# MJavaadAkhtar/GCN-max-cut

Measured on AMD Instinct MI355X. Metric: training epochs/sec (n=1000 d=7 graphs), higher is better.
Workload: dtype f32; 1 GPU; 160 x n=1000 d=7 regular graphs per GPU (BASELINE configs[3] on one GPU; 160 graphs per step), GCN 1000->500->3, batched steps, Adam lr 1e-3; graphs_per_gpu=160, rows_per_gpu=160000, nnz_per_gpu=1120000, hidden_dim=500, mode=batched, epoch_graphs=160, parallelism=single

## Files before the change

gcn-max-cut_amd/csrc/bwd1_lds.hip:

```cpp
#include "lds_tile.h"
#include "head_body.h"

#ifdef GMC_STAMP
extern "C" int gmc_debug_read_stamps_bwd(unsigned long long *out, int n) {
    return (int)hipMemcpyFromSymbol(out, HIP_SYMBOL(g_stamps), sizeof(unsigned long long) * n);
}
extern "C" int gmc_debug_read_stamps_bwdhead(unsigned long long *out, int n) {
    return (int)hipMemcpyFromSymbol(out, HIP_SYMBOL(g_hstamps), sizeof(unsigned long long) * n);
}
#endif

namespace {

struct Bwd1Args {
    gmc_batch b;
    const float *H;
    const float *GY2;
    const float *W2;
    float *dw1part;
    float *colpart;
    int F;
    int slices;
    int chunks;
    int graphs_per_chunk;
    int ovf_cap;
    int own_lds;
    const float *hZ0;
    int hzparts;
    float hC;
    const float *hb2;
    float *hP;
    int *hS;
    float *hloss;
    float *hdb2part;
    int *htick;
};

struct ColState {
    gmc::v2f w2p[2][3];
    gmc::v2f cdw2[3][2], cdb1[2];
};

__device__ __forceinline__ void col_state_init(ColState &c, const float *W2, int f0, bool col_on) {
#pragma unroll
    for (int p = 0; p < 2; ++p) {
#pragma unroll
        for (int k = 0; k < 3; ++k) {
            c.w2p[p][k] = col_on ? (gmc::v2f){W2[(long)(f0 + 2 * p) * 3 + k], W2[(long)(f0 + 2 * p + 1) * 3 + k]}
                                 : gmc::splat2(0.f);
            c.cdw2[k][p] = gmc::splat2(0.f);
        }
        c.cdb1[p] = gmc::splat2(0.f);
    }
}

__device__ __forceinline__ void transform_row(ColState &c, float4 *cell, const float4 rck, const float4 *hreg = nullptr) {
    const float d = rck.w;
    const float4 h = hreg ? *hreg : *cell;
    const gmc::v2f g0 = gmc::splat2(rck.x * d), g1 = gmc::splat2(rck.y * d), g2 = gmc::splat2(rck.z * d);
    const gmc::v2f hp[2] = {{h.x, h.y}, {h.z, h.w}};
    gmc::v2f gs[2];
#pragma unroll
    for (int p = 0; p < 2; ++p) {
        gmc::v2f ghd = g0 * c.w2p[p][0];
        ghd = gmc::pk_fma(g1, c.w2p[p][1], ghd);
        ghd = gmc::pk_fma(g2, c.w2p[p][2], ghd);
        const gmc::v2f gpre = {hp[p].x > 0.f ? ghd.x : 0.f, hp[p].y > 0.f ? ghd.y : 0.f};
        gs[p] = gpre * gmc::splat2(d);
        if (ABL(3)) continue;
        c.cdw2[0][p] = gmc::pk_fma(hp[p], g0, c.cdw2[0][p]);
        c.cdw2[1][p] = gmc::pk_fma(hp[p], g1, c.cdw2[1][p]);
        c.cdw2[2][p] = gmc::pk_fma(hp[p], g2, c.cdw2[2][p]);
        c.cdb1[p] += gpre;
    }
    *cell = make_float4(gs[0].x, gs[0].y, gs[1].x, gs[1].y);
#pragma unroll
    for (int p = 0; p < 2; ++p)
        asm volatile("" : "+v"(c.cdw2[0][p]), "+v"(c.cdw2[1][p]), "+v"(c.cdw2[2][p]), "+v"(c.cdb1[p]));
}

template <int Q>
__device__ __forceinline__ void col_epilogue(const ColState &c, float *red, float *colpart, int chunk, int s, int FS, int F) {
    float colp[16];
#pragma unroll
    for (int p = 0; p < 2; ++p) {
#pragma unroll
        for (int k = 0; k < 3; ++k) { colp[4 * (2 * p) + k] = c.cdw2[k][p].x; colp[4 * (2 * p + 1) + k] = c.cdw2[k][p].y; }
        colp[4 * (2 * p) + 3] = c.cdb1[p].x; colp[4 * (2 * p + 1) + 3] = c.cdb1[p].y;
    }
#pragma unroll
    for (int i = 0; i < 16; ++i) colp[i] = gmc::xor_tree<32, Q>(colp[i]);
    const int wave = threadIdx.x >> 6, lane = threadIdx.x & 63;
    if (lane < Q) {
#pragma unroll
        for (int i = 0; i < 16; ++i) red[(wave * Q + lane) * 16 + i] = colp[i];
    }
    lds_barrier();
    if (threadIdx.x < Q * 4) {
        const int qq = threadIdx.x / 4, j = threadIdx.x % 4;
        if (s * FS + 4 * qq < F) {
            float o[4] = {0.f, 0.f, 0.f, 0.f};
            for (int wv = 0; wv < kThreads / 64; ++wv)
#pragma unroll
                for (int cc = 0; cc < 4; ++cc) o[cc] += red[(wv * Q + qq) * 16 + 4 * j + cc];
            reinterpret_cast<float4 *>(colpart)[(long)chunk * F + s * FS + 4 * qq + j] = make_float4(o[0], o[1], o[2], o[3]);
        }
    }
}

__device__ __forceinline__ void dma_row_consts(const float *GY2, int r0, int n, float *gyl) {
    const unsigned base = (unsigned)(size_t)(__attribute__((address_space(3))) float *)gyl;
    int tid = threadIdx.x;
    asm volatile("" : "+v"(tid));
    for (int i0 = 0; i0 < n; i0 += kThreads) {
        const unsigned dst = (unsigned)__builtin_amdgcn_readfirstlane((int)(base + 16u * (unsigned)(i0 + (tid & ~63))));
        if (i0 + tid < n) glds16(GY2 + (long)(r0 + i0 + tid) * 4, dst);
    }
}

template <int FS, int ACC, bool HAS_VAL, int NS, bool OVF, bool HEAD = false>
__global__ GMC_LDS_BOUNDS void bwd1_reg_kernel(Bwd1Args a) {
    extern __shared__ __attribute__((aligned(16))) float lds[];
    constexpr int W = 8;
    constexpr int Q = FS / 4;
    constexpr int kRowsPerPass = kThreads / Q;
    int chunk, s;
    MARK(0);
    tile_of((int)blockIdx.x, a.chunks, a.slices, chunk, s);
    const int TF = (int)tile_floats(a.b.n_max, FS);
    float *bufA = lds, *bufB = lds + TF;
    float *gy0 = lds + 2 * TF + (size_t)a.b.n_max * W / 2;
    float *gy1 = lds + 2 * TF;
    float *red = bufB;
    const int q = threadIdx.x % Q, lrow = threadIdx.x / Q;
    const int f0 = s * FS + 4 * q;
    const bool col_on = f0 < a.F;
    const float *Hs = a.H + (long)s * a.b.R * FS;
    ColState cs;
    col_state_init(cs, a.W2, f0, col_on);
    gmc::v4f acc[ACC];
#pragma unroll
    for (int k = 0; k < ACC; ++k) acc[k] = (gmc::v4f)(0.f);

    const int g0 = chunk * a.graphs_per_chunk, g1 = min(a.b.B, g0 + a.graphs_per_chunk);
    if (g0 >= g1) return;
    constexpr bool ovf = OVF;

    constexpr bool kRecycle = !HAS_VAL && !OVF;
    constexpr int KREG = kRecycle ? 3 : 0;
    float4 hreg[kRecycle ? KREG : 1];
    auto load_cell = [&](int slot, int k, int r0n, int nn) {
        const int l = min(lrow + k * kRowsPerPass, nn - 1);
        const gmc::v4f v = __builtin_nontemporal_load(reinterpret_cast<const gmc::v4f *>(Hs + (long)(r0n + l) * FS + 4 * q));
        hreg[slot] = make_float4(v.x, v.y, v.z, v.w);
    };
    auto load_hreg = [&](int r0n, int nn) {
#pragma unroll
        for (int k = 0; k < KREG; ++k) {
            const int l = min(lrow + k * kRowsPerPass, nn - 1);
            const gmc::v4f v = __builtin_nontemporal_load(reinterpret_cast<const gmc::v4f *>(Hs + (long)(r0n + l) * FS + 4 * q));
            hreg[k] = make_float4(v.x, v.y, v.z, v.w);
        }
    };
    uint4 idr[ACC];
    OvfLds ol{};
    constexpr int kOvfRows = (ACC * kRowsPerPass + kThreads - 1) / kThreads;
    OvfReq<kOvfRows> orq;
    if constexpr (ovf) ol = ovf_lds(lds, a.own_lds, a.b.n_max, a.ovf_cap);
    auto load_ids = [&](int r0, int n) {
#pragma unroll
        for (int k = 0; k < ACC; ++k)
            idr[k] = *reinterpret_cast<const uint4 *>(a.b.ell + (long)(r0 + min(lrow + k * kRowsPerPass, n - 1)) * W);
    };
    auto pad_ids = [&](int n) {
        const unsigned pad = (unsigned)n * 0x10001u;
#pragma unroll
        for (int k = 0; k < ACC; ++k)
            if (lrow + k * kRowsPerPass >= n) idr[k] = make_uint4(pad, pad, pad, pad);
    };
    auto zero_pads = [&](float *buf, int n) {
        if (threadIdx.x < kPadRows * FS) buf[n * FS + threadIdx.x] = 0.f;
    };
    auto fetch_tile = [&](int r0, int n) {
        constexpr int kRows = kThreads / (FS / 4);
        const unsigned base = (unsigned)(size_t)(__attribute__((address_space(3))) float *)bufA;
        const unsigned wave_dst = (unsigned)__builtin_amdgcn_readfirstlane((int)(base + 16u * (threadIdx.x & ~63u)));
#pragma unroll
        for (int k = 0; k < ACC; ++k) {
            const int l = lrow + k * kRows;
            if (l < n) glds16<true>(Hs + (long)(r0 + l) * FS + 4 * q, wave_dst + 16u * (unsigned)(k * kThreads));
        }
    };
    auto row_consts = [&](int k, int n, const float *gyl) {
        return reinterpret_cast<const float4 *>(gyl)[min(lrow + k * kRowsPerPass, n - 1)];
    };
    auto transform_with = [&](int k, int n, float4 rck) {
        if (ABL(7)) return;
        const int l = lrow + k * kRowsPerPass;
        if (l >= n) rck = gmc::f4_zero();
        transform_row(cs, reinterpret_cast<float4 *>(bufA) + min(l, n) * Q + q, rck, kRecycle ? &hreg[k % KREG] : nullptr);
    };
    auto transform = [&](int k, int n, const float *gyl) { transform_with(k, n, row_consts(k, n, gyl)); };

    int r0 = a.b.goff[g0], n = a.b.goff[g0 + 1] - r0;
    int nn = g0 + 1 < g1 ? a.b.goff[g0 + 2] - (r0 + n) : 0;
    if constexpr (!HEAD) dma_row_consts(a.GY2, r0, n, gy0);
    if (!kRecycle) fetch_tile(r0, n);
    load_hreg(r0, n);
    float4 hlast = gmc::f4_zero();
    if constexpr (kRecycle && ACC == KREG + 1) {
        const int l = min(lrow + (ACC - 1) * kRowsPerPass, n - 1);
        const gmc::v4f v = __builtin_nontemporal_load(reinterpret_cast<const gmc::v4f *>(Hs + (long)(r0 + l) * FS + 4 * q));
        hlast = make_float4(v.x, v.y, v.z, v.w);
    }
    load_ids(r0, n);
    if constexpr (ovf) ovf_setup<kOvfRows>(a.b, r0, n, ol);
    if constexpr (HEAD) {
        static_assert(kThreads == kHeadThreads && !HAS_VAL && !OVF, "one-graph unit-weight launches only");
        const HeadArgs ha{a.b, a.hZ0, a.hzparts, a.hb2, a.hC, a.hP, a.hS, a.hloss, nullptr, a.hdb2part, a.htick};
        head_body<8>(ha, g0, bufB, blockIdx.x == 0, reinterpret_cast<float4 *>(gy0));
    }
    zero_pads(bufA, n);
    dma_wait();
    __syncthreads();
    STAMP_DECL;
    MARK(1);
    if constexpr (kRecycle && ACC == KREG + 1) {
#pragma unroll
        for (int k = 0; k < KREG; ++k) transform(k, n, gy0);
        hreg[0] = hlast;
        transform(ACC - 1, n, gy0);
    } else {
#pragma unroll
        for (int k = 0; k < ACC; ++k) {
            transform(k, n, gy0);
            if (kRecycle && k + KREG < ACC) load_cell(k % KREG, k + KREG, r0, n);
        }
    }
    for (int g = g0; g < g1; ++g) {
        const int cur = (g - g0) & 1;
        const float *gyl = cur ? gy1 : gy0;
        float *gyn = cur ? gy0 : gy1;
        const int r0n = r0 + n;
        STAMP(0);
#pragma unroll
        for (int k = 0; k < ACC; ++k) asm volatile("" : "+v"(idr[k].x), "+v"(idr[k].y), "+v"(idr[k].z), "+v"(idr[k].w));
        pad_ids(n);
        if (nn > 0 && !ABL(1)) dma_row_consts(a.GY2, r0n, nn, gyn);
        STAMP(1);
        loop_barrier();
        STAMP(2);
        if (kRecycle) load_hreg(nn > 0 ? r0n : r0, nn > 0 ? nn : n);
        unsigned hd[ovf ? ACC : 1] = {};
        bool hub_any = false;
        if constexpr (ovf) {
#pragma unroll
            for (int k = 0; k < ACC; ++k) hd[k] = ovf_desc(ol, min(lrow + k * kRowsPerPass, n - 1));
            unsigned any = 0;
#pragma unroll
            for (int k = 0; k < ACC; ++k) {
                if (lrow + k * kRowsPerPass >= n) hd[k] = 0;
                any |= hd[k];
            }
            hub_any = __builtin_amdgcn_ballot_w64(any != 0) != 0;
        }
        zero_pads(bufB, n);
        float dv[ACC];
#pragma unroll
        for (int k = 0; k < ACC; ++k) dv[k] = gyl[4 * min(lrow + k * kRowsPerPass, n - 1) + 3];
#pragma unroll
        for (int k = 0; k < ACC; ++k) {
            const int l = min(lrow + k * kRowsPerPass, n);
            float4 u;
            if constexpr (ovf) u = gather_ids8_halves<FS>(bufA, idr[k], q);
            else u = ABL(5) ? make_float4(dv[k], dv[k], dv[k], dv[k]) : gather_ids8<FS, false, NS>(bufA, idr[k], nullptr, q);
            u.x *= dv[k]; u.y *= dv[k]; u.z *= dv[k]; u.w *= dv[k];
            reinterpret_cast<float4 *>(bufB)[l * Q + q] = u;
        }
        if (hub_any) {
#pragma unroll
            for (int k = 0; k < ACC; ++k) {
                const int lm = lrow + k * kRowsPerPass;
                float4 mine = gmc::f4_zero();
                for_hub_rows<FS, 0>(hd[k], lm, q, bufA, nullptr, ol, n, [&](int l, const float4 t) { if (lm == l) mine = t; });
                if (hd[k] != 0) {
                    float4 *cell = reinterpret_cast<float4 *>(bufB) + lm * Q + q;
                    const float4 c = *cell;
                    *cell = make_float4(fmaf(mine.x, dv[k], c.x), fmaf(mine.y, dv[k], c.y), fmaf(mine.z, dv[k], c.z), fmaf(mine.w, dv[k], c.w));
                }
            }
        }
        STAMP(3);
        if (kRecycle) vm_wait<KREG>();
        else dma_wait();
        loop_barrier();
        STAMP(4);
        if (kRecycle) {
            if (nn > 0) zero_pads(bufA, nn);
        } else if (nn > 0 && !ABL(1)) {
            fetch_tile(r0n, nn);
            zero_pads(bufA, nn);
            if constexpr (ovf) ovf_request(a.b, r0n, nn, (int)threadIdx.x, orq);
        }
        STAMP(5);
        const float *wbase = HAS_VAL ? a.b.ell_vals + (long)r0 * W : nullptr;
#pragma unroll
        for (int k = 0; k < 2 * ACC; ++k) {
            if (k < ACC) {
                if (kRecycle && nn > 0) {
                    transform(k, nn, gyn);
                    if (k + KREG < ACC) load_cell(k % KREG, k + KREG, r0n, nn);
                }
                const int l = min(lrow + k * kRowsPerPass, n - 1);
                if constexpr (HAS_VAL) acc[k] += gmc::f4v(gather_ids8<FS, true, NS>(bufB, idr[k], wbase + (long)l * W, q));
                else if constexpr (ovf) acc[k] += gmc::f4v(gather_ids8_halves<FS>(bufB, idr[k], q));
                else acc[k] += ABL(4) ? (gmc::v4f)(__uint_as_float(idr[k].x)) : gather_ids8_pk<FS, NS>(bufB, idr[k], q);
                asm volatile("" : "+v"(acc[k]));
                if (k == ACC - 1 && nn > 0) load_ids(r0n, nn);
            }
            if (!kRecycle && k >= ACC && nn > 0) {
                const int j = k - ACC;
                if (j == 0) vm_wait<ACC>();
                __builtin_amdgcn_sched_barrier(0);
                transform(j, nn, gyn);
            }
        }
        if constexpr (ovf) {
            if (nn > 0 && !ABL(1)) ovf_blocks(a.b, (int)threadIdx.x, ol, orq);
        }
        if (hub_any) {
#pragma unroll
            for (int k = 0; k < ACC; ++k) {
                const int lm = lrow + k * kRowsPerPass;
                for_hub_rows<FS, 0>(hd[k], lm, q, bufB, nullptr, ol, n, [&](int l, const float4 t) { if (lm == l) acc[k] += gmc::f4v(t); });
            }
        }
        STAMP(6);
        STAMP(7);
        if constexpr (ovf) {
            if (nn > 0) {
                loop_barrier();
                ovf_commit(a.b, nn, (int)threadIdx.x, ol, orq);
            }
        }
        STAMP(9);
        const int n2 = g + 2 < g1 ? sload(a.b.goff, g + 3) - (r0n + nn) : 0;
        r0 = r0n; n = nn; nn = n2;
    }
    STAMP_FLUSH;
    MARK(2);
    if (col_on) {
#pragma unroll
        for (int k = 0; k < ACC; ++k) {
            const int l = lrow + k * kRowsPerPass;
            if (l < a.b.n_max) *reinterpret_cast<float4 *>(a.dw1part + ((long)chunk * a.b.n_max + l) * a.F + f0) = gmc::v4f_f4(acc[k]);
        }
    }
    lds_barrier();
    col_epilogue<Q>(cs, red, a.colpart, chunk, s, FS, a.F);
    MARK(3);
}

template <int FS, int W, int ACC, bool HAS_VAL, int NS, bool OVF>
__global__ GMC_LDS_BOUNDS void bwd1_lds_kernel(Bwd1Args a) {
    extern __shared__ __attribute__((aligned(16))) float lds[];
    constexpr int Q = FS / 4;
    constexpr int kRowsPerPass = kThreads / Q;
    constexpr int NT = (ACC * kRowsPerPass * (W / 8) + kThreads - 1) / kThreads;
    constexpr int RC = (ACC * kRowsPerPass + kThreads - 1) / kThreads;
    int chunk, s;
    tile_of((int)blockIdx.x, a.chunks, a.slices, chunk, s);
    const int TF = (int)tile_floats(a.b.n_max, FS);
    float *bufA = lds, *bufB = lds + TF;
    unsigned short *nb = reinterpret_cast<unsigned short *>(lds + 2 * TF);
    float4 *gyl = reinterpret_cast<float4 *>(bufB);
    float *red = bufB;
    const int q = threadIdx.x % Q, lrow = threadIdx.x / Q;
    const int f0 = s * FS + 4 * q;
    const bool col_on = f0 < a.F;
    const long slab = (long)s * a.b.R * FS;
    constexpr bool ovf = OVF;
    ColState cs;
    col_state_init(cs, a.W2, f0, col_on);
    gmc::v4f acc[ACC];
    uint4 pt[NT];
    float4 rc[RC];
    OvfLds ol{};
    OvfReq<RC> orq;
    if constexpr (ovf) ol = ovf_lds(lds, a.own_lds, a.b.n_max, a.ovf_cap);
#pragma unroll
    for (int k = 0; k < ACC; ++k) acc[k] = (gmc::v4f)(0.f);

    const int g0 = chunk * a.graphs_per_chunk, g1 = min(a.b.B, g0 + a.graphs_per_chunk);
    if (g0 >= g1) return;
    auto fetch = [&](int r0, int n) {
        dma_tile<FS, ACC, true>(a.H + slab + (long)r0 * FS + 4 * q, FS, n, true, lrow, bufA);
        const uint4 *src = reinterpret_cast<const uint4 *>(a.b.ell + (long)r0 * W);
#pragma unroll
        for (int k = 0; k < NT; ++k) {
            const int i = threadIdx.x + k * kThreads;
            pt[k] = i < n * (W / 8) ? src[i] : make_uint4(0, 0, 0, 0);
        }
#pragma unroll
        for (int k = 0; k < RC; ++k) {
            const int i = threadIdx.x + k * kThreads;
            rc[k] = reinterpret_cast<const float4 *>(a.GY2)[r0 + min(i, n - 1)];
        }
        if constexpr (ovf) ovf_request(a.b, r0, n, (int)threadIdx.x, orq);
    };
    auto commit = [&](int r0, int n) {
#pragma unroll
        for (int k = 0; k < NT; ++k) {
            const int i = threadIdx.x + k * kThreads;
            if (i < n * (W / 8)) reinterpret_cast<uint4 *>(nb)[i] = pt[k];
        }
#pragma unroll
        for (int k = 0; k < RC; ++k) {
            const int i = threadIdx.x + k * kThreads;
            if (i < n) gyl[i] = rc[k];
        }
        if (threadIdx.x < kPadRows * FS) {
            bufA[n * FS + threadIdx.x] = 0.f;
            bufB[n * FS + threadIdx.x] = 0.f;
        }
        if constexpr (ovf) ovf_commit(a.b, n, (int)threadIdx.x, ol, orq);
    };
    int r0 = a.b.goff[g0], n = a.b.goff[g0 + 1] - r0;
    fetch(r0, n);
    if constexpr (ovf) ovf_blocks(a.b, (int)threadIdx.x, ol, orq);
    commit(r0, n);
    dma_wait();
    __syncthreads();
    for (int g = g0; g < g1; ++g) {
        const int r0n = r0 + n;
        const int nn = g + 1 < g1 ? sload(a.b.goff, g + 2) - r0n : n;
        float dv[ACC];
        unsigned hub = 0;
        bool hub_any = false;
        if constexpr (ovf) {
            unsigned d[ACC];
#pragma unroll
            for (int k = 0; k < ACC; ++k) d[k] = ovf_desc(ol, min(lrow + k * kRowsPerPass, n - 1));
#pragma unroll
            for (int k = 0; k < ACC; ++k) hub |= (d[k] != 0 && lrow + k * kRowsPerPass < n ? 1u : 0u) << k;
            hub_any = __builtin_amdgcn_ballot_w64(hub != 0) != 0;
        }
#pragma unroll
        for (int k = 0; k < ACC; ++k) {
            const int l = lrow + k * kRowsPerPass;
            const float4 rck = gyl[min(l, n - 1)];
            dv[k] = rck.w;
            transform_row(cs, reinterpret_cast<float4 *>(bufA) + min(l, n) * Q + q, rck);
        }
        __syncthreads();
#pragma unroll
        for (int k = 0; k < ACC; ++k) {
            const int l = lrow + k * kRowsPerPass;
            if (l < n) {
                float4 u = gather_row<FS, W, false, NS>(bufA, nb, nullptr, l, q);
                u.x *= dv[k]; u.y *= dv[k]; u.z *= dv[k]; u.w *= dv[k];
                reinterpret_cast<float4 *>(bufB)[l * Q + q] = u;
            }
        }
        if (hub_any) {
#pragma unroll
            for (int k = 0; k < ACC; ++k) {
                const int lm = lrow + k * kRowsPerPass;
                const unsigned hdk = (hub >> k & 1u) ? ovf_desc(ol, lm) : 0u;
                float4 mine = gmc::f4_zero();
                for_hub_rows<FS, 0>(hdk, lm, q, bufA, nullptr, ol, n, [&](int l, const float4 t) { if (lm == l) mine = t; });
                if (hdk != 0) {
                    float4 *cell = reinterpret_cast<float4 *>(bufB) + lm * Q + q;
                    const float4 c = *cell;
                    *cell = make_float4(fmaf(mine.x, dv[k], c.x), fmaf(mine.y, dv[k], c.y), fmaf(mine.z, dv[k], c.z), fmaf(mine.w, dv[k], c.w));
                }
            }
        }
        __syncthreads();
        if (g + 1 < g1) fetch(r0n, nn);
        const float *wbase = HAS_VAL ? a.b.ell_vals + (long)r0 * W : nullptr;
#pragma unroll
        for (int k = 0; k < ACC; ++k) {
            const int l = lrow + k * kRowsPerPass;
            if (l < n) {
                acc[k] += gmc::f4v(gather_row<FS, W, HAS_VAL, NS>(bufB, nb, HAS_VAL ? wbase + (long)l * W : nullptr, l, q));
                asm volatile("" : "+v"(acc[k]));
            }
        }
        if (hub_any) {
#pragma unroll
            for (int k = 0; k < ACC; ++k) {
                const int lm = lrow + k * kRowsPerPass;
                const unsigned hdk = (hub >> k & 1u) ? ovf_desc(ol, lm) : 0u;
                for_hub_rows<FS, 0>(hdk, lm, q, bufB, nullptr, ol, n, [&](int l, const float4 t) { if (lm == l) acc[k] += gmc::f4v(t); });
            }
        }
        dma_wait();
        if constexpr (ovf) {
            if (g + 1 < g1) ovf_blocks(a.b, (int)threadIdx.x, ol, orq);
        }
        __syncthreads();
        if (g + 1 < g1) commit(r0n, nn);
        __syncthreads();
        r0 = r0n; n = nn;
    }
    if (col_on) {
#pragma unroll
        for (int k = 0; k < ACC; ++k) {
            const int l = lrow + k * kRowsPerPass;
            if (l < a.b.n_max) *reinterpret_cast<float4 *>(a.dw1part + ((long)chunk * a.b.n_max + l) * a.F + f0) = gmc::v4f_f4(acc[k]);
        }
    }
    col_epilogue<Q>(cs, red, a.colpart, chunk, s, FS, a.F);
}

struct Bwd1Built {
    template <typename L> static constexpr bool has(L) {
        if (L::EPI || L::SHARED || (L::HAS_VAL && L::OVF)) return false;
        if (L::HEAD) return L::W == 8 && L::ACC == 4 && !L::HAS_VAL && !L::OVF;
        return L::HAS_VAL || L::OVF ? L::NS == L::W : true;
    }
};

}

bool gmc_bwd1_takes_head(const gmc_batch *b) {
    if (!b || b->B != 1 || b->ell_width != 8 || b->ell_vals || gmc_has_overflow(b) || !gmc_lds_fits(b)) return false;
    const int fs = pick_fs(b->n_max, b->ell_width);
    const int rows_per_pass = kThreads / (fs / 4);
    if (b->n_max > 4 * rows_per_pass || b->n_max > kHeadThreads) return false;
    return (size_t)(7 * (b->n_max + 4) + 64) <= tile_floats(b->n_max, fs);
}

int gmc_bwd1_flavour(const gmc_batch *b, int F, bool head) {
    const GmcLdsGeom g = gmc_lds_geometry(b, F);
    if (!g.fits || F <= 0) return 0;
    if (head && !gmc_bwd1_takes_head(b)) return 0;
    return flavour_word(g.W == 8 ? GMC_FLV_BWD1_REG : GMC_FLV_BWD1, g.fs, g.W, g.acc, g.hv, g.ns, g.ovf, head);
}

int gmc_bwd1_lds_launch(const gmc_batch *b, const float *H, const float *GY2, const float *W2,
                        float *dw1part, float *colpart, int F, int chunks, int graphs_per_chunk,
                        hipStream_t st, const gmc_bwd1_head *head) {
    const int flv = gmc_bwd1_flavour(b, F, head != nullptr);
    if (!flv) return GMC_ERR_UNSUPPORTED;
    if (head && (chunks != 1 || !head->Z0 || !head->b2 || !head->P || !head->db2part)) return GMC_ERR_UNSUPPORTED;
    const int fs = GMC_FLV_FS(flv);
    Bwd1Args a{*b, H, GY2, W2, dw1part, colpart, F, (F + fs - 1) / fs, chunks, graphs_per_chunk, 0, 0,
               head ? head->Z0 : nullptr, head ? head->zparts : 0, head ? head->C : 0.f, head ? head->b2 : nullptr,
               head ? head->P : nullptr, head ? head->S : nullptr, head ? head->loss : nullptr,
               head ? head->db2part : nullptr, head ? head->tick : nullptr};
    size_t lds = lds_bytes(b->n_max, b->ell_width, fs);
    if (gmc_has_overflow(b)) {
        const size_t own = ovf_own_bytes(1, b->n_max, b->ell_width, fs);
        if (own + ovf_desc_bytes(b->n_max) > kOvfLdsBytes) return GMC_ERR_UNSUPPORTED;
        a.own_lds = (int)own;
        a.ovf_cap = ovf_cap_blocks(own, b->n_max);
        lds = kOvfLdsBytes;
    }
    GmcProbeScope probe(GMC_K_BWD1_FUSED, st);
    return decode_flavour<Bwd1Built>(flv, [&](auto L) {
        using K = decltype(L);
        const int grid = a.slices * a.chunks;
        if constexpr (K::W == 8)
            return launch_flv(flv, K::word(GMC_FLV_BWD1_REG), bwd1_reg_kernel<K::FS, K::ACC, K::HAS_VAL, K::NS, K::OVF, K::HEAD>,
                              grid, lds, st, a);
        else
            return launch_flv(flv, K::word(GMC_FLV_BWD1), bwd1_lds_kernel<K::FS, K::W, K::ACC, K::HAS_VAL, K::NS, K::OVF>,
                              grid, lds, st, a);
    });
}
```

gcn-max-cut_amd/csrc/head.hip:

```cpp
#include "head_body.h"
#include "launchers.h"

#ifdef GMC_STAMP
extern "C" int gmc_debug_read_stamps_head(unsigned long long *out, int n) {
    return (int)hipMemcpyFromSymbol(out, HIP_SYMBOL(g_hstamps), sizeof(unsigned long long) * n);
}
#endif

namespace {

template <int W>
__global__ __launch_bounds__(kHeadThreads) void head_kernel(HeadArgs a) {
    extern __shared__ __attribute__((aligned(16))) float lds[];
    head_body<W>(a, (int)blockIdx.x, lds, true, nullptr);
}

template <int W>
__global__ __launch_bounds__(kHeadThreads) void head_soft_kernel(HeadArgs a) {
    extern __shared__ __attribute__((aligned(16))) float lds[];
    head_body<W, true>(a, (int)blockIdx.x, lds, true, nullptr);
}

struct HeadBwdArgs {
    gmc_batch b;
    const float *P;
    const float *GP;
    float *GY2;
    float *db2part;
};

__global__ __launch_bounds__(kHeadThreads) void head_bwd_kernel(HeadBwdArgs a) {
    extern __shared__ __attribute__((aligned(16))) float lds[];
    const int g = blockIdx.x;
    const int r0 = a.b.goff[g];
    const int n = a.b.goff[g + 1] - r0;
    float *sA = lds;
    float *red = lds + 3 * a.b.n_max;
    float acc[4] = {0.f, 0.f, 0.f, 0.f};
    for (int l = threadIdx.x; l < n; l += blockDim.x) {
        const long r = r0 + l;
        const float g0 = a.GP[r * 3], g1 = a.GP[r * 3 + 1], g2 = a.GP[r * 3 + 2];
        const float p0 = a.P[r * 3], p1 = a.P[r * 3 + 1], p2 = a.P[r * 3 + 2];
        const float dot = g0 * p0 + g1 * p1 + g2 * p2;
        const float z0 = p0 * (g0 - dot), z1 = p1 * (g1 - dot), z2 = p2 * (g2 - dot);
        acc[1] += z0; acc[2] += z1; acc[3] += z2;
        const float d = a.b.dinv[r];
        sA[3 * l] = z0 * d; sA[3 * l + 1] = z1 * d; sA[3 * l + 2] = z2 * d;
    }
    block_sum4(acc, red);
    if (threadIdx.x == 0) {
        a.db2part[g * 3] = acc[1]; a.db2part[g * 3 + 1] = acc[2]; a.db2part[g * 3 + 2] = acc[3];
    }
    for (int l = threadIdx.x; l < n; l += blockDim.x) {
        const int r = r0 + l;
        const int beg = a.b.rowptr[r], end = a.b.rowptr[r + 1];
        float y0 = 0.f, y1 = 0.f, y2 = 0.f;
        for (int e = beg; e < end; ++e) {
            const int c = a.b.lcol[e];
            y0 += sA[3 * c]; y1 += sA[3 * c + 1]; y2 += sA[3 * c + 2];
        }
        *reinterpret_cast<float4 *>(a.GY2 + (long)r * 4) = make_float4(y0, y1, y2, a.b.dinv[r]);
    }
}

int check_batch(const gmc_batch *b) {
    if (!b) return GMC_ERR_NULL;
    if (b->abi != GMC_VERSION) return GMC_ERR_ABI;
    if (!b->goff || !b->rowptr || !b->gcol || !b->lcol || !b->dinv) return GMC_ERR_NULL;
    if (b->B < 0 || b->R < 0 || b->nnz < 0) return GMC_ERR_SHAPE;
    if (b->B > 0 && (b->n_max < 3 || b->n_max > GMC_MAX_GRAPH_NODES)) return GMC_ERR_GRAPH_SIZE;
    return GMC_OK;
}

}

extern "C" int gmc_head_f32(const gmc_batch *batch, const float *Z0, int32_t z_parts, const float *b2,
                            float C, float *P, int32_t *S, float *loss, float *GY2, float *db2part,
                            gmc_stream_t stream) {
    return gmc_head_launch(batch, Z0, z_parts, b2, C, P, S, loss, GY2, db2part, nullptr,
                           static_cast<hipStream_t>(stream), GMC_LOSS_CUT);
}

extern "C" int gmc_head_loss_f32(const gmc_batch *batch, const float *Z0, int32_t z_parts, const float *b2,
                                 float C, int32_t loss_kind, float *P, int32_t *S, float *loss, float *GY2,
                                 float *db2part, gmc_stream_t stream) {
    if (!gmc_loss_kind_ok(loss_kind)) return GMC_ERR_LOSS;
    return gmc_head_launch(batch, Z0, z_parts, b2, C, P, S, loss, GY2, db2part, nullptr,
                           static_cast<hipStream_t>(stream), loss_kind);
}

int gmc_head_launch(const gmc_batch *batch, const float *Z0, int32_t z_parts, const float *b2, float C, float *P,
                    int32_t *S, float *loss, float *GY2, float *db2part, int *tick, hipStream_t stream, int loss_kind) {
    int rc = check_batch(batch);
    if (rc) return rc;
    if (!Z0 || !b2 || !P) return GMC_ERR_NULL;
    if (z_parts < 1) return GMC_ERR_SHAPE;
    if (GY2 && !db2part) return GMC_ERR_NULL;
    if (batch->B == 0) return GMC_OK;
    HeadArgs a{*batch, Z0, z_parts, b2, C, P, S, loss, GY2, db2part, tick};
    const bool soft = loss_kind == GMC_LOSS_EXPECTED_CUT;
    const size_t lds = sizeof(float) * (7 * ((size_t)batch->n_max + 4) + 64 + (soft ? 12 : 0));
    const int w = (batch->ell != nullptr && (batch->ell_width == 8 || batch->ell_width == 16)) ? batch->ell_width : 0;
    const void *fn = soft ? (w == 8 ? reinterpret_cast<const void *>(head_soft_kernel<8>)
                             : w == 16 ? reinterpret_cast<const void *>(head_soft_kernel<16>)
                                       : reinterpret_cast<const void *>(head_soft_kernel<0>))
                   : w == 8 ? reinterpret_cast<const void *>(head_kernel<8>)
                   : w == 16 ? reinterpret_cast<const void *>(head_kernel<16>) : reinterpret_cast<const void *>(head_kernel<0>);
    if (lds > 64 * 1024) {
        hipError_t e = hipFuncSetAttribute(fn, hipFuncAttributeMaxDynamicSharedMemorySize, (int)lds);
        if (e != hipSuccess) return (int)e;
    }
    GmcProbeScope probe(GMC_K_HEAD, stream);
    if (soft) {
        if (w == 8) hipLaunchKernelGGL(head_soft_kernel<8>, dim3(batch->B), dim3(kHeadThreads), lds, stream, a);
        else if (w == 16) hipLaunchKernelGGL(head_soft_kernel<16>, dim3(batch->B), dim3(kHeadThreads), lds, stream, a);
        else hipLaunchKernelGGL(head_soft_kernel<0>, dim3(batch->B), dim3(kHeadThreads), lds, stream, a);
    } else if (w == 8) hipLaunchKernelGGL(head_kernel<8>, dim3(batch->B), dim3(kHeadThreads), lds, stream, a);
    else if (w == 16) hipLaunchKernelGGL(head_kernel<16>, dim3(batch->B), dim3(kHeadThreads), lds, stream, a);
    else hipLaunchKernelGGL(head_kernel<0>, dim3(batch->B), dim3(kHeadThreads), lds, stream, a);
    GMC_LAUNCH_CHECK();
    return GMC_OK;
}

int gmc_head_bwd_launch(const gmc_batch *batch, const float *P, const float *GP, float *GY2,
                        float *db2part, hipStream_t st) {
    int rc = check_batch(batch);
    if (rc) return rc;
    if (batch->B == 0) return GMC_OK;
    HeadBwdArgs a{*batch, P, GP, GY2, db2part};
    const size_t lds = sizeof(float) * (3 * (size_t)batch->n_max + 64);
    GmcProbeScope probe(GMC_K_HEAD, st);
    hipLaunchKernelGGL(head_bwd_kernel, dim3(batch->B), dim3(kHeadThreads), lds, st, a);
    GMC_LAUNCH_CHECK();
    return GMC_OK;
}
```

gcn-max-cut_amd/csrc/head_body.h:

```cpp
#pragma once
#include "gmc_common.h"

#ifdef GMC_STAMP
static __device__ unsigned long long g_hstamps[2 * 16];
#define HMARK(i)                                                                                         \
    do {                                                                                                 \
        __builtin_amdgcn_sched_barrier(0);                                                               \
        if (blockIdx.x == 0 && (threadIdx.x == 0 || threadIdx.x == kHeadThreads - 64))                   \
            g_hstamps[(threadIdx.x ? 16 : 0) + (i)] = __builtin_amdgcn_s_memrealtime();                  \
        __builtin_amdgcn_sched_barrier(0);                                                               \
    } while (0)
#else
#define HMARK(i)
#endif

namespace {

constexpr int kHeadThreads = 1024;

struct HeadArgs {
    gmc_batch b;
    const float *Z0;
    int zparts;
    const float *b2;
    float C;
    float *P;
    int *S;
    float *loss;
    float *GY2;
    float *db2part;
    int *tick;
};

__device__ __forceinline__ void block_sum4(float (&v)[4], float *red ) {
    const int lane = gmc::lane_id(), wave = threadIdx.x >> 6;
#pragma unroll
    for (int k = 0; k < 4; ++k) v[k] = gmc::wave_sum(v[k]);
    if (lane == 0) {
#pragma unroll
        for (int k = 0; k < 4; ++k) red[wave * 4 + k] = v[k];
    }
    __syncthreads();
    if (threadIdx.x == 0) {
        float part[kHeadThreads / 64][4];
#pragma unroll
        for (int w = 0; w < kHeadThreads / 64; ++w)
#pragma unroll
            for (int k = 0; k < 4; ++k) part[w][k] = red[w * 4 + k];
        float s0 = 0.f, s1 = 0.f, s2 = 0.f, s3 = 0.f;
#pragma unroll
        for (int w = 0; w < kHeadThreads / 64; ++w) { s0 += part[w][0]; s1 += part[w][1]; s2 += part[w][2]; s3 += part[w][3]; }
        v[0] = s0; v[1] = s1; v[2] = s2; v[3] = s3;
    }
}

template <int W, typename F>
__device__ __forceinline__ void for_neighbours(const gmc_batch &b, int r0, int l, int n, bool cached, const uint4 c0,
                                               const uint4 c1, F &&f) {
    if constexpr (W > 0) {
        const uint4 *row = reinterpret_cast<const uint4 *>(b.ell + (long)(r0 + l) * W);
#pragma unroll
        for (int blk = 0; blk < W / 8; ++blk) {
            const uint4 ids = cached ? (blk == 0 ? c0 : c1) : row[blk];
            const unsigned pk[4] = {ids.x, ids.y, ids.z, ids.w};
#pragma unroll
            for (int u = 0; u < 8; ++u) {
                const unsigned id = (u & 1) ? pk[u >> 1] >> 16 : pk[u >> 1] & 0xffffu;
                f((int)id, b.ell_vals ? b.ell_vals[(long)(r0 + l) * W + blk * 8 + u] : 1.0f);
            }
        }
        if (b.ovf_ptr) {
            for (int blk = b.ovf_ptr[r0 + l]; blk < b.ovf_ptr[r0 + l + 1]; ++blk) {
                const uint4 ids = reinterpret_cast<const uint4 *>(b.ovf_ids)[blk];
                const unsigned pk[4] = {ids.x, ids.y, ids.z, ids.w};
#pragma unroll
                for (int u = 0; u < 8; ++u) {
                    const unsigned id = (u & 1) ? pk[u >> 1] >> 16 : pk[u >> 1] & 0xffffu;
                    f((int)id, b.ovf_vals ? b.ovf_vals[8l * blk + u] : 1.0f);
                }
            }
        }
    } else {
        for (int e = b.rowptr[r0 + l]; e < b.rowptr[r0 + l + 1]; ++e) f(b.lcol[e], b.vals ? b.vals[e] : 1.0f);
    }
    (void)n;
}

template <int W, bool SOFT = false>
__device__ __forceinline__ void head_body(const HeadArgs &a, const int g, float *lds, const bool outputs, float4 *gy_lds) {
    constexpr bool ELL = W > 0;
    HMARK(0);
    const int r0 = a.b.goff[g];
    const int n = a.b.goff[g + 1] - r0;
    const int NP = a.b.n_max + 4;
    float *sA = lds;
    float *sP = lds + 3 * NP;
    int *sS = reinterpret_cast<int *>(lds + 6 * NP);
    float *red = lds + 7 * NP;
    float *sT = red + 64;
    const bool train = a.GY2 != nullptr || gy_lds != nullptr;
    if (a.tick && outputs && g == 0 && threadIdx.x == 0) (void)__hip_atomic_fetch_add(a.tick, 1, __ATOMIC_RELAXED, __HIP_MEMORY_SCOPE_AGENT);

    const int l0 = threadIdx.x;
    uint4 cid0 = make_uint4(0, 0, 0, 0), cid1 = cid0;
    float cd = 0.f;
    if (l0 < n) {
        cd = a.b.dinv[r0 + l0];
        if (ELL) {
            const uint4 *row = reinterpret_cast<const uint4 *>(a.b.ell + (long)(r0 + l0) * W);
            cid0 = row[0];
            if (W > 8) cid1 = row[1];
        }
    }
    const float bias0 = a.b2[0], bias1 = a.b2[1], bias2 = a.b2[2];
    constexpr int kFoldElems = 3, kFoldRound = 16;
    for (int i0 = threadIdx.x; i0 < 3 * n; i0 += kFoldElems * (int)blockDim.x) {
        float z[kFoldElems] = {};
        int ie[kFoldElems];
#pragma unroll
        for (int e = 0; e < kFoldElems; ++e) ie[e] = min(i0 + e * (int)blockDim.x, 3 * n - 1);
        for (int p0 = 0; p0 < a.zparts; p0 += kFoldRound) {
            float t[kFoldElems][kFoldRound];
#pragma unroll
            for (int u = 0; u < kFoldRound; ++u) {
                const float *zu = a.Z0 + ((long)min(p0 + u, a.zparts - 1) * a.b.R + r0) * 3;
#pragma unroll
                for (int e = 0; e < kFoldElems; ++e) t[e][u] = zu[ie[e]];
            }
#pragma unroll
            for (int e = 0; e < kFoldElems; ++e)
#pragma unroll
                for (int u = 0; u < kFoldRound; ++u) z[e] += p0 + u < a.zparts ? t[e][u] : 0.f;
        }
#pragma unroll
        for (int e = 0; e < kFoldElems; ++e) {
            const int i = i0 + e * (int)blockDim.x;
            if (i < 3 * n) sA[i] = z[e];
        }
    }
    if (threadIdx.x < 12) sA[3 * n + threadIdx.x] = 0.f;
    if (threadIdx.x < 4) sS[n + threadIdx.x] = 3;
    if constexpr (SOFT) {
        if (threadIdx.x < 12) sP[3 * n + threadIdx.x] = 0.f;
    }
    HMARK(1);
    __syncthreads();
    HMARK(2);

    for (int l = threadIdx.x; l < n; l += blockDim.x) {
        const int r = r0 + l;
        float z0 = 0.f, z1 = 0.f, z2 = 0.f;
        for_neighbours<W>(a.b, r0, l, n, l == l0, cid0, cid1, [&](int c, float) { z0 += sA[3 * c]; z1 += sA[3 * c + 1]; z2 += sA[3 * c + 2]; });
        const float d = l == l0 ? cd : a.b.dinv[r];
        z0 = fmaf(z0, d, bias0); z1 = fmaf(z1, d, bias1); z2 = fmaf(z2, d, bias2);
        const float m = fmaxf(z0, fmaxf(z1, z2));
        const float e0 = expf(z0 - m), e1 = expf(z1 - m), e2 = expf(z2 - m);
        const float inv = 1.0f / (e0 + e1 + e2);
        const float p0 = e0 * inv, p1 = e1 * inv, p2 = e2 * inv;
        if (outputs) { a.P[(long)r * 3] = p0; a.P[(long)r * 3 + 1] = p1; a.P[(long)r * 3 + 2] = p2; }
        if (SOFT && l < 3) {
            sT[3 * l] = p0; sT[3 * l + 1] = p1; sT[3 * l + 2] = p2;
            sP[3 * l] = l == 0 ? 1.f : 0.f; sP[3 * l + 1] = l == 1 ? 1.f : 0.f; sP[3 * l + 2] = l == 2 ? 1.f : 0.f;
        } else {
            sP[3 * l] = p0; sP[3 * l + 1] = p1; sP[3 * l + 2] = p2;
        }
        int s;
        if (l < 3) {
            s = l;
        } else {
            s = 0;
            float best = p0;
            if (p1 > best) { best = p1; s = 1; }
            if (p2 > best) { s = 2; }
        }
        sS[l] = s;
        if (a.S && outputs) a.S[r] = s;
    }
    HMARK(3);
    __syncthreads();
    HMARK(4);

    float acc[4] = {0.f, 0.f, 0.f, 0.f};
    for (int l = threadIdx.x; l < n; l += blockDim.x) {
        const int r = r0 + l;
        const int me = sS[l];
        float g0 = 0.f, g1 = 0.f, g2 = 0.f, cut = 0.f;
        if constexpr (SOFT) {
            const float u0 = sP[3 * l], u1 = sP[3 * l + 1], u2 = sP[3 * l + 2];
            for_neighbours<W>(a.b, r0, l, n, l == l0, cid0, cid1, [&](int c, float w) {
                const float q0 = sP[3 * c], q1 = sP[3 * c + 1], q2 = sP[3 * c + 2];
                const float wv = c < n ? w : 0.f;
                g0 += wv * q0; g1 += wv * q1; g2 += wv * q2;
                cut += wv * (1.0f - (u0 * q0 + u1 * q1 + u2 * q2));
            });
        } else {
            for_neighbours<W>(a.b, r0, l, n, l == l0, cid0, cid1, [&](int c, float w) {
                const int sc = sS[c];
                g0 += sc == 0 ? w : 0.f; g1 += sc == 1 ? w : 0.f; g2 += sc == 2 ? w : 0.f;
                cut += (sc != me && sc != 3) ? w : 0.f;
            });
        }
        acc[0] += cut;
        if (train) {
            g0 *= a.C; g1 *= a.C; g2 *= a.C;
            const bool own = SOFT && l < 3;
            const float p0 = own ? sT[3 * l] : sP[3 * l], p1 = own ? sT[3 * l + 1] : sP[3 * l + 1],
                        p2 = own ? sT[3 * l + 2] : sP[3 * l + 2];
            const float dot = g0 * p0 + g1 * p1 + g2 * p2;
            const float z0 = p0 * (g0 - dot), z1 = p1 * (g1 - dot), z2 = p2 * (g2 - dot);
            acc[1] += z0; acc[2] += z1; acc[3] += z2;
            const float d = l == l0 ? cd : a.b.dinv[r];
            sA[3 * l] = z0 * d; sA[3 * l + 1] = z1 * d; sA[3 * l + 2] = z2 * d;
        }
    }
    HMARK(5);
    block_sum4(acc, red);
    HMARK(6);
    if (threadIdx.x == 0 && outputs) {
        if (a.loss) __hip_atomic_store(a.loss + g, -a.C * (acc[0] * 0.5f), __ATOMIC_RELAXED, __HIP_MEMORY_SCOPE_SYSTEM);
        if (train && a.db2part) {
            a.db2part[g * 3] = acc[1]; a.db2part[g * 3 + 1] = acc[2]; a.db2part[g * 3 + 2] = acc[3];
        }
    }
    if (!train) return;
    HMARK(7);

    for (int l = threadIdx.x; l < n; l += blockDim.x) {
        const int r = r0 + l;
        float y0 = 0.f, y1 = 0.f, y2 = 0.f;
        for_neighbours<W>(a.b, r0, l, n, l == l0, cid0, cid1, [&](int c, float) { y0 += sA[3 * c]; y1 += sA[3 * c + 1]; y2 += sA[3 * c + 2]; });
        const float4 row = make_float4(y0, y1, y2, l == l0 ? cd : a.b.dinv[r]);
        if (gy_lds) gy_lds[l] = row;
        else *reinterpret_cast<float4 *>(a.GY2 + (long)r * 4) = row;
    }
    HMARK(8);
#ifdef GMC_STAMP
    __builtin_amdgcn_s_waitcnt(0);
    HMARK(9);
#endif
}

}
```

Before: 3783 epochs/s (1 epoch = 160 graphs).

## Pad head LDS arrays to float4 rows and precompute neighbour LDS addresses

```diff
diff --git a/gcn-max-cut_amd/csrc/bwd1_lds.hip b/gcn-max-cut_amd/csrc/bwd1_lds.hip
--- a/gcn-max-cut_amd/csrc/bwd1_lds.hip
+++ b/gcn-max-cut_amd/csrc/bwd1_lds.hip
@@ -529,7 +529,7 @@
     const int fs = pick_fs(b->n_max, b->ell_width);
     const int rows_per_pass = kThreads / (fs / 4);
     if (b->n_max > 4 * rows_per_pass || b->n_max > kHeadThreads) return false;
-    return (size_t)(7 * (b->n_max + 4) + 64) <= tile_floats(b->n_max, fs);
+    return head_lds_floats(b->n_max, false) <= tile_floats(b->n_max, fs);
 }
 
 int gmc_bwd1_flavour(const gmc_batch *b, int F, bool head) {
diff --git a/gcn-max-cut_amd/csrc/head.hip b/gcn-max-cut_amd/csrc/head.hip
--- a/gcn-max-cut_amd/csrc/head.hip
+++ b/gcn-max-cut_amd/csrc/head.hip
@@ -99,7 +99,7 @@
     if (batch->B == 0) return GMC_OK;
     HeadArgs a{*batch, Z0, z_parts, b2, C, P, S, loss, GY2, db2part, tick};
     const bool soft = loss_kind == GMC_LOSS_EXPECTED_CUT;
-    const size_t lds = sizeof(float) * (7 * ((size_t)batch->n_max + 4) + 64 + (soft ? 12 : 0));
+    const size_t lds = sizeof(float) * head_lds_floats(batch->n_max, soft);
     const int w = (batch->ell != nullptr && (batch->ell_width == 8 || batch->ell_width == 16)) ? batch->ell_width : 0;
     const void *fn = soft ? (w == 8 ? reinterpret_cast<const void *>(head_soft_kernel<8>)
                              : w == 16 ? reinterpret_cast<const void *>(head_soft_kernel<16>)
diff --git a/gcn-max-cut_amd/csrc/head_body.h b/gcn-max-cut_amd/csrc/head_body.h
--- a/gcn-max-cut_amd/csrc/head_body.h
+++ b/gcn-max-cut_amd/csrc/head_body.h
@@ -86,6 +86,56 @@
     (void)n;
 }
 
+typedef float head_v4f __attribute__((ext_vector_type(4)));
+__device__ __forceinline__ head_v4f lds_row16(unsigned addr) {
+    return *(__attribute__((address_space(3))) const head_v4f *)(size_t)addr;
+}
+__device__ __forceinline__ int lds_word(unsigned addr) {
+    return *(__attribute__((address_space(3))) const int *)(size_t)addr;
+}
+__device__ __forceinline__ void row_addrs8(const uint4 ids, unsigned base, unsigned *ad) {
+    const unsigned pk[4] = {ids.x, ids.y, ids.z, ids.w};
+#pragma unroll
+    for (int j = 0; j < 4; ++j) {
+        asm("v_mad_u32_u16 %0, %1, 16, %2" : "=v"(ad[2 * j]) : "v"(pk[j]), "v"(base));
+        asm("v_mad_u32_u16 %0, %1, 16, %2 op_sel:[1,0,0,0]" : "=v"(ad[2 * j + 1]) : "v"(pk[j]), "v"(base));
+    }
+}
+template <int W, bool FAST, typename F>
+__device__ __forceinline__ void for_neighbour_rows(const gmc_batch &b, int r0, int l, unsigned base,
+                                                   const unsigned (&off)[W > 0 ? W : 1], F &&f) {
+    if constexpr (W > 0) {
+        const uint4 *row = reinterpret_cast<const uint4 *>(b.ell + (long)(r0 + l) * W);
+#pragma unroll
+        for (int blk = 0; blk < W / 8; ++blk) {
+            unsigned ad[8];
+            if constexpr (FAST) {
+#pragma unroll
+                for (int u = 0; u < 8; ++u) ad[u] = off[blk * 8 + u];
+            } else {
+                row_addrs8(row[blk], base, ad);
+            }
+#pragma unroll
+            for (int u = 0; u < 8; ++u) f(ad[u], b.ell_vals ? b.ell_vals[(long)(r0 + l) * W + blk * 8 + u] : 1.0f);
+        }
+        if (b.ovf_ptr) {
+            for (int blk = b.ovf_ptr[r0 + l]; blk < b.ovf_ptr[r0 + l + 1]; ++blk) {
+                unsigned ad[8];
+                row_addrs8(reinterpret_cast<const uint4 *>(b.ovf_ids)[blk], base, ad);
+#pragma unroll
+                for (int u = 0; u < 8; ++u) f(ad[u], b.ovf_vals ? b.ovf_vals[8l * blk + u] : 1.0f);
+            }
+        }
+    } else {
+        for (int e = b.rowptr[r0 + l]; e < b.rowptr[r0 + l + 1]; ++e) f(base + 16u * (unsigned)b.lcol[e], b.vals ? b.vals[e] : 1.0f);
+    }
+}
+
+struct HeadFastRow { static constexpr bool value = true; };
+struct HeadSlowRow { static constexpr bool value = false; };
+
+__host__ __device__ inline size_t head_lds_floats(int n_max, bool soft) { return 8 * ((size_t)n_max + 4) + 64 + (soft ? 12 : 0); }
+
 template <int W, bool SOFT = false>
 __device__ __forceinline__ void head_body(const HeadArgs &a, const int g, float *lds, const bool outputs, float4 *gy_lds) {
     constexpr bool ELL = W > 0;
@@ -93,11 +143,12 @@
     const int r0 = a.b.goff[g];
     const int n = a.b.goff[g + 1] - r0;
     const int NP = a.b.n_max + 4;
-    float *sA = lds;
-    float *sP = lds + 3 * NP;
-    int *sS = reinterpret_cast<int *>(lds + 6 * NP);
-    float *red = lds + 7 * NP;
+    float4 *sA = reinterpret_cast<float4 *>(lds);
+    float4 *sP = sA + NP;
+    float *red = lds + 8 * NP;
     float *sT = red + 64;
+    const unsigned baseA = (unsigned)(size_t)(__attribute__((address_space(3))) float *)lds;
+    const unsigned dP = 16u * (unsigned)NP, dS = dP + 12u;
     const bool train = a.GY2 != nullptr || gy_lds != nullptr;
     if (a.tick && outputs && g == 0 && threadIdx.x == 0) (void)__hip_atomic_fetch_add(a.tick, 1, __ATOMIC_RELAXED, __HIP_MEMORY_SCOPE_AGENT);
 
@@ -135,35 +186,37 @@
 #pragma unroll
         for (int e = 0; e < kFoldElems; ++e) {
             const int i = i0 + e * (int)blockDim.x;
-            if (i < 3 * n) sA[i] = z[e];
-        }
-    }
-    if (threadIdx.x < 12) sA[3 * n + threadIdx.x] = 0.f;
-    if (threadIdx.x < 4) sS[n + threadIdx.x] = 3;
-    if constexpr (SOFT) {
-        if (threadIdx.x < 12) sP[3 * n + threadIdx.x] = 0.f;
+            if (i < 3 * n) lds[i + i / 3] = z[e];
+        }
+    }
+    if (threadIdx.x < 4) {
+        sA[n + threadIdx.x] = make_float4(0.f, 0.f, 0.f, 0.f);
+        sP[n + threadIdx.x] = make_float4(0.f, 0.f, 0.f, __int_as_float(3));
+    }
+    unsigned off[ELL ? W : 1] = {};
+    if constexpr (ELL) {
+        row_addrs8(cid0, baseA, off);
+        if constexpr (W > 8) row_addrs8(cid1, baseA, off + 8);
     }
     HMARK(1);
     __syncthreads();
     HMARK(2);
 
-    for (int l = threadIdx.x; l < n; l += blockDim.x) {
+    auto phase1 = [&](const int l, auto fast) {
+        constexpr bool FAST = decltype(fast)::value;
         const int r = r0 + l;
         float z0 = 0.f, z1 = 0.f, z2 = 0.f;
-        for_neighbours<W>(a.b, r0, l, n, l == l0, cid0, cid1, [&](int c, float) { z0 += sA[3 * c]; z1 += sA[3 * c + 1]; z2 += sA[3 * c + 2]; });
-        const float d = l == l0 ? cd : a.b.dinv[r];
+        for_neighbour_rows<W, FAST>(a.b, r0, l, baseA, off, [&](unsigned ad, float) {
+            const head_v4f v = lds_row16(ad);
+            z0 += v.x; z1 += v.y; z2 += v.z;
+        });
+        const float d = FAST ? cd : a.b.dinv[r];
         z0 = fmaf(z0, d, bias0); z1 = fmaf(z1, d, bias1); z2 = fmaf(z2, d, bias2);
         const float m = fmaxf(z0, fmaxf(z1, z2));
         const float e0 = expf(z0 - m), e1 = expf(z1 - m), e2 = expf(z2 - m);
         const float inv = 1.0f / (e0 + e1 + e2);
         const float p0 = e0 * inv, p1 = e1 * inv, p2 = e2 * inv;
         if (outputs) { a.P[(long)r * 3] = p0; a.P[(long)r * 3 + 1] = p1; a.P[(long)r * 3 + 2] = p2; }
-        if (SOFT && l < 3) {
-            sT[3 * l] = p0; sT[3 * l + 1] = p1; sT[3 * l + 2] = p2;
-            sP[3 * l] = l == 0 ? 1.f : 0.f; sP[3 * l + 1] = l == 1 ? 1.f : 0.f; sP[3 * l + 2] = l == 2 ? 1.f : 0.f;
-        } else {
-            sP[3 * l] = p0; sP[3 * l + 1] = p1; sP[3 * l + 2] = p2;
-        }
         int s;
         if (l < 3) {
             s = l;
@@ -173,29 +226,40 @@
             if (p1 > best) { best = p1; s = 1; }
             if (p2 > best) { s = 2; }
         }
-        sS[l] = s;
+        if (SOFT && l < 3) {
+            sT[3 * l] = p0; sT[3 * l + 1] = p1; sT[3 * l + 2] = p2;
+            sP[l] = make_float4(l == 0 ? 1.f : 0.f, l == 1 ? 1.f : 0.f, l == 2 ? 1.f : 0.f, __int_as_float(s));
+        } else {
+            sP[l] = make_float4(p0, p1, p2, __int_as_float(s));
+        }
         if (a.S && outputs) a.S[r] = s;
-    }
+    };
+    if (l0 < n) phase1(l0, HeadFastRow{});
+    for (int l = l0 + (int)blockDim.x; l < n; l += blockDim.x) phase1(l, HeadSlowRow{});
     HMARK(3);
     __syncthreads();
     HMARK(4);
 
     float acc[4] = {0.f, 0.f, 0.f, 0.f};
-    for (int l = threadIdx.x; l < n; l += blockDim.x) {
+    auto phase2 = [&](const int l, auto fast) {
+        constexpr bool FAST = decltype(fast)::value;
         const int r = r0 + l;
-        const int me = sS[l];
+        const float4 own = sP[l];
         float g0 = 0.f, g1 = 0.f, g2 = 0.f, cut = 0.f;
         if constexpr (SOFT) {
-            const float u0 = sP[3 * l], u1 = sP[3 * l + 1], u2 = sP[3 * l + 2];
-            for_neighbours<W>(a.b, r0, l, n, l == l0, cid0, cid1, [&](int c, float w) {
-                const float q0 = sP[3 * c], q1 = sP[3 * c + 1], q2 = sP[3 * c + 2];
-                const float wv = c < n ? w : 0.f;
+            const float u0 = own.x, u1 = own.y, u2 = own.z;
+            const unsigned pad = baseA + 16u * (unsigned)n;
+            for_neighbour_rows<W, FAST>(a.b, r0, l, baseA, off, [&](unsigned ad, float w) {
+                const head_v4f qv = lds_row16(ad + dP);
+                const float q0 = qv.x, q1 = qv.y, q2 = qv.z;
+                const float wv = ad < pad ? w : 0.f;
                 g0 += wv * q0; g1 += wv * q1; g2 += wv * q2;
                 cut += wv * (1.0f - (u0 * q0 + u1 * q1 + u2 * q2));
             });
         } else {
-            for_neighbours<W>(a.b, r0, l, n, l == l0, cid0, cid1, [&](int c, float w) {
-                const int sc = sS[c];
+            const int me = __float_as_int(own.w);
+            for_neighbour_rows<W, FAST>(a.b, r0, l, baseA, off, [&](unsigned ad, float w) {
+                const int sc = lds_word(ad + dS);
                 g0 += sc == 0 ? w : 0.f; g1 += sc == 1 ? w : 0.f; g2 += sc == 2 ? w : 0.f;
                 cut += (sc != me && sc != 3) ? w : 0.f;
             });
@@ -203,16 +267,17 @@
         acc[0] += cut;
         if (train) {
             g0 *= a.C; g1 *= a.C; g2 *= a.C;
-            const bool own = SOFT && l < 3;
-            const float p0 = own ? sT[3 * l] : sP[3 * l], p1 = own ? sT[3 * l + 1] : sP[3 * l + 1],
-                        p2 = own ? sT[3 * l + 2] : sP[3 * l + 2];
+            const bool mine = SOFT && l < 3;
+            const float p0 = mine ? sT[3 * l] : own.x, p1 = mine ? sT[3 * l + 1] : own.y, p2 = mine ? sT[3 * l + 2] : own.z;
             const float dot = g0 * p0 + g1 * p1 + g2 * p2;
             const float z0 = p0 * (g0 - dot), z1 = p1 * (g1 - dot), z2 = p2 * (g2 - dot);
             acc[1] += z0; acc[2] += z1; acc[3] += z2;
-            const float d = l == l0 ? cd : a.b.dinv[r];
-            sA[3 * l] = z0 * d; sA[3 * l + 1] = z1 * d; sA[3 * l + 2] = z2 * d;
-        }
-    }
+            const float d = FAST ? cd : a.b.dinv[r];
+            sA[l] = make_float4(z0 * d, z1 * d, z2 * d, 0.f);
+        }
+    };
+    if (l0 < n) phase2(l0, HeadFastRow{});
+    for (int l = l0 + (int)blockDim.x; l < n; l += blockDim.x) phase2(l, HeadSlowRow{});
     HMARK(5);
     block_sum4(acc, red);
     HMARK(6);
@@ -225,14 +290,20 @@
     if (!train) return;
     HMARK(7);
 
-    for (int l = threadIdx.x; l < n; l += blockDim.x) {
+    auto phase3 = [&](const int l, auto fast) {
+        constexpr bool FAST = decltype(fast)::value;
         const int r = r0 + l;
         float y0 = 0.f, y1 = 0.f, y2 = 0.f;
-        for_neighbours<W>(a.b, r0, l, n, l == l0, cid0, cid1, [&](int c, float) { y0 += sA[3 * c]; y1 += sA[3 * c + 1]; y2 += sA[3 * c + 2]; });
-        const float4 row = make_float4(y0, y1, y2, l == l0 ? cd : a.b.dinv[r]);
+        for_neighbour_rows<W, FAST>(a.b, r0, l, baseA, off, [&](unsigned ad, float) {
+            const head_v4f v = lds_row16(ad);
+            y0 += v.x; y1 += v.y; y2 += v.z;
+        });
+        const float4 row = make_float4(y0, y1, y2, FAST ? cd : a.b.dinv[r]);
         if (gy_lds) gy_lds[l] = row;
         else *reinterpret_cast<float4 *>(a.GY2 + (long)r * 4) = row;
-    }
+    };
+    if (l0 < n) phase3(l0, HeadFastRow{});
+    for (int l = l0 + (int)blockDim.x; l < n; l += blockDim.x) phase3(l, HeadSlowRow{});
     HMARK(8);
 #ifdef GMC_STAMP
     __builtin_amdgcn_s_waitcnt(0);
```

Result: no change. 3805 epochs/s (1 epoch = 160 graphs) (median of 5 runs) (+0.6%).
